# LeonardoTemperanza/LupinPathTracer

Hardware: AMD Instinct MI355X
Metric: Msamples/sec (paths x bounces) (higher is better)
Workload: dtype f32; 1 GPU; bistro_class 3840x2160, 16 bounces, 8 spp per step, Standard integrator, software BVH (BASELINE configs[4] frame; stand-in scene for bistroexterior, SURVEY 8d); frames_in_flight=1, frames_per_wavefront=6, first_pass_stack_entries=26, traversal=binary

## Files before the change

### lupinpathtracer_amd/csrc/lupin_hip.hip

```cpp

#include <hip/hip_runtime.h>
#include <hip/hip_fp16.h>
#include <cstdio>
#include <cstdlib>
#include <cstring>
#include <cmath>
#include <string>
#include <vector>
#include <set>
#include <mutex>
#include <algorithm>
#include <atomic>

#include "lupin_stages.hpp"
#include "lupin_denoise.hpp"
#include "lupin_adaptive.hpp"
#include "lupin_internal.hpp"


static inline float host_u2f(uint32_t u) { float f; memcpy(&f, &u, 4); return f; }

static thread_local std::string g_last_error;
static int fail(int code, const std::string &msg) { g_last_error = msg; return code; }
#define HIP_TRY(expr) do { hipError_t e__ = (expr); if (e__ != hipSuccess) return fail(LUPIN_ERR_HIP, std::string(#expr) + ": " + hipGetErrorString(e__)); } while (0)
// ... 88 lines not shown

struct LupinDoubleBufferedTexture
{
    LupinContext *ctx;
    LupinTexture *tex[2];
    int front_idx, back_idx;
};

struct LupinScene
{
    LupinContext *ctx;
    int device = 0;
    SceneDev dev{};
    std::vector<void *> allocations;
    uint32_t stack_entries = 1;
    uint32_t persistent_blocks[2][4] = {{0, 0, 0, 0}, {0, 0, 0, 0}};
    uint32_t wide_blocks[4] = {0, 0, 0, 0};
    uint32_t short_blocks[4] = {0, 0, 0, 0};
    bool has_wide = false;
    uint64_t leaky_triangles = 0;
    uint64_t id = 0;
    bool all_opaque = false;
    bool simple_matte = false;
    bool has_sw_bvh = false;
    bool envs_empty = true, lights_empty = true, instances_empty = true;
};

template <typename T>
static int upload(LupinScene *sc, const std::vector<T> &host, const T **out)
{
    *out = nullptr;
    size_t bytes = std::max<size_t>(host.size() * sizeof(T), sizeof(T) > 16 ? sizeof(T) : 16);
    void *d = nullptr;
    HIP_TRY(hipMalloc(&d, bytes));
    sc->allocations.push_back(d);
    HIP_TRY(hipMemsetAsync(d, 0, bytes, sc->ctx->stream));
    if (!host.empty()) HIP_TRY(hipMemcpyAsync(d, host.data(), host.size() * sizeof(T), hipMemcpyHostToDevice, sc->ctx->stream));
    *out = reinterpret_cast<const T *>(d);
    return LUPIN_OK;
}

static hipEvent_t get_event(LupinContext *ctx)
{
    if (!ctx->ev_pool.empty()) { hipEvent_t e = ctx->ev_pool.back(); ctx->ev_pool.pop_back(); return e; }
    hipEvent_t e = nullptr;
    hipEventCreate(&e);
    return e;
}

static void set_path_layout(Lane *ln, bool records)
{
    PathBuffers &pb = ln->pb;
    char *b = ln->hot;
    const size_t cap = (size_t)ln->capacity;
    pb.skey = {ln->skey, 4};
    if (records)
    {
        const uint32_t st = LP_PATH_RECORD_BYTES;
        pb.ori_rng = {b + 0, st}; pb.dir_meta = {b + 16, st}; pb.hit = {b + 32, st}; pb.hit_tri = {b + 48, st};
        pb.weight = {b + 64, st}; pb.radiance = {b + 80, st}; pb.color = {b + 96, st};
        char *m = ln->shadow;
        pb.sh_org = {m + 0, st}; pb.sh_d0 = {m + 16, st}; pb.sh_d1 = {m + 32, st}; pb.next_tri = {m + 48, st};
        pb.sh_f0 = {m + 64, st}; pb.sh_f1 = {m + 80, st}; pb.next_hit = {m + 96, st}; pb.sh_hit1 = {m + 112, st};
    }
    else
    {
        pb.ori_rng = {b, 16}; pb.dir_meta = {b + 16 * cap, 16}; pb.hit = {b + 32 * cap, 16}; pb.weight = {b + 48 * cap, 16};
        pb.radiance = {b + 64 * cap, 16}; pb.color = {b + 80 * cap, 16}; pb.hit_tri = {b + 96 * cap, 4};
        char *m = ln->shadow;
        pb.sh_org = {m, 16}; pb.sh_d0 = {m + 16 * cap, 16}; pb.sh_d1 = {m + 32 * cap, 16}; pb.sh_f0 = {m + 48 * cap, 16};
        pb.sh_f1 = {m + 64 * cap, 16}; pb.next_hit = {m + 80 * cap, 16}; pb.sh_hit1 = {m + 96 * cap, 16}; pb.next_tri = {m + 112 * cap, 4};
    }
}

static int ensure_path_buffers(LupinContext *ctx0, Lane *ctx, uint64_t slots, uint32_t iterations)
{
    (void)ctx0;
    const uint64_t per_round = (uint64_t)LP_SHARDS * LP_BLOCK;
    slots = (slots + per_round - 1) / per_round * per_round;
    if (slots > ctx->capacity)
    {
        PathBuffers &pb = ctx->pb;
        void **ptrs[] = {(void **)&ctx->hot, (void **)&ctx->shadow, (void **)&ctx->skey, (void **)&pb.vol0, (void **)&pb.vol1, (void **)&pb.queue[0], (void **)&pb.queue[1],
                         (void **)&pb.retrace};
        size_t elem[] = {LP_PATH_RECORD_BYTES, LP_PATH_RECORD_BYTES, 4, 16, 16, 4, 4, 8};
        constexpr int NPTRS = 8;
        HIP_TRY(hipStreamSynchronize(ctx->stream));
        ctx->capacity = 0;
        ctx->pb_generation++;
        for (int k = 0; k < NPTRS; k++)
            if (*ptrs[k]) { hipFree(*ptrs[k]); *ptrs[k] = nullptr; }
        for (int k = 0; k < NPTRS; k++)
            HIP_TRY(hipMalloc(ptrs[k], (size_t)slots * elem[k]));
        for (int k = 0; k < NPTRS; k++)
            HIP_TRY(hipMemsetAsync(*ptrs[k], 0, (size_t)slots * elem[k], ctx->stream));
        ctx->capacity = slots;
    }
    if (iterations + 2 > ctx->counts_capacity)
    {
        HIP_TRY(hipStreamSynchronize(ctx->stream));
        ctx->counts_capacity = 0;
        if (ctx->pb.counts) hipFree(ctx->pb.counts);
        ctx->pb.counts = nullptr;
        ctx->pb.cursors = ctx->pb.retrace_counts = ctx->pb.retrace_cursors = nullptr;
        HIP_TRY(hipMalloc((void **)&ctx->pb.counts, LP_COUNTER_ROWS * (size_t)(iterations + 2) * LP_SHARDS * sizeof(uint32_t)));
        ctx->counts_capacity = iterations + 2;
        ctx->pb.cursors = ctx->pb.counts + (size_t)ctx->counts_capacity * LP_SHARDS;
        ctx->pb.retrace_counts = ctx->pb.cursors + 2 * (size_t)ctx->counts_capacity * LP_SHARDS;
        ctx->pb.retrace_cursors = ctx->pb.retrace_counts + 2 * (size_t)ctx->counts_capacity * LP_SHARDS;
        ctx->pb_generation++;
    }
    return LUPIN_OK;
}

static uint32_t collapse_to_wide4(const std::vector<WideNode> &bin, uint32_t root_ref, std::vector<Wide4> &out, uint32_t *out_depth = nullptr)
{
    if (out_depth) *out_depth = 0;
    if (root_ref & REF_LEAF) return root_ref;
    struct Child { float lo[3], hi[3]; uint32_t ref; bool leaky, closed; };
    auto children_of = [&](uint32_t b, Child &l, Child &r) {
        const WideNode &w = bin[b];
        l.lo[0] = w.a.x; l.lo[1] = w.a.z; l.lo[2] = w.b.x; l.hi[0] = w.b.z; l.hi[1] = w.c.x; l.hi[2] = w.c.z; l.ref = w.d.x;
        r.lo[0] = w.a.y; r.lo[1] = w.a.w; r.lo[2] = w.b.y; r.hi[0] = w.b.w; r.hi[1] = w.c.y; r.hi[2] = w.c.w; r.ref = w.d.y;
        l.leaky = (w.d.z & 1u) != 0; r.leaky = (w.d.z & 2u) != 0;
        l.closed = r.closed = false;
    };
    auto inside = [](const Child &in, const Child &out) {
        for (int ax = 0; ax < 3; ax++)
            if (!(in.lo[ax] >= out.lo[ax] && in.hi[ax] <= out.hi[ax])) return false;
        return true;
    };
    auto area = [](const Child &c) {
        const double ex = (double)c.hi[0] - c.lo[0], ey = (double)c.hi[1] - c.lo[1], ez = (double)c.hi[2] - c.lo[2];
        const double a = ex * ey + ey * ez + ez * ex;
        return a == a ? a : 0.0;
    };
    struct Item { uint32_t bin_node, wide_node, depth; };
    std::vector<Item> todo;
    const uint32_t root = (uint32_t)out.size();
    out.emplace_back();
    todo.push_back({root_ref, root, 1u});
    const float nanf_ = std::nanf("");
    while (!todo.empty())
    {
        const Item it = todo.back();
        todo.pop_back();
        if (out_depth) *out_depth = std::max(*out_depth, it.depth);
        Child c[4];
        int n = 2;
        children_of(it.bin_node, c[0], c[1]);
        while (n < 4)
        {
            int pick = -1;
            double best = -1.0;
            for (int k = 0; k < n; k++)
                if (!(c[k].ref & REF_LEAF) && !c[k].closed) { const double a = area(c[k]); if (a > best) { best = a; pick = k; } }
            if (pick < 0) break;
            Child l, r;
            children_of(c[pick].ref, l, r);
            if (!inside(l, c[pick]) || !inside(r, c[pick])) { c[pick].closed = true; continue; }
            c[pick] = l;
            c[n++] = r;
        }
        Wide4 w;
        float *lo[3] = {&w.lox.x, &w.loy.x, &w.loz.x}, *hi[3] = {&w.hix.x, &w.hiy.x, &w.hiz.x};
        uint32_t refs[4];
        for (int k = 0; k < 4; k++)
        {
            for (int ax = 0; ax < 3; ax++) { lo[ax][k] = k < n ? c[k].lo[ax] : nanf_; hi[ax][k] = k < n ? c[k].hi[ax] : nanf_; }
// ... 256 lines not shown
template <int TYPE, int MODE>
static void launch_persistent_tracer(LupinContext *ctx, Lane *ln, const LupinScene *scene, const Shape &sh, uint32_t iter)
{
    hipStream_t st = ln->stream;
    const FrameParams *fp = ln->d_fp;
    unsigned long long *work = ln->work_counters, *wide = ln->wide_counters;
    {
        if (sh.wblocks)
        {
            if (ctx->counting)
            {
                hipLaunchKernelGGL((k_extend_persistent<TYPE, false, MODE, true, true, false>), dim3(sh.wblocks), dim3(LP_BLOCK), sh.wlds, st,
                                   scene->dev, fp, ln->pb, iter, ln->stat_counters, LP_REFILL_MIN, sh.wstack_words, LP_NODE_STEPS, work, wide);
                hipLaunchKernelGGL((k_extend_persistent<TYPE, false, MODE, true, false, true>), dim3(sh.pblocks), dim3(LP_BLOCK), sh.lds, st,
                                   scene->dev, fp, ln->pb, iter, ln->stat_counters, LP_REFILL_MIN, sh.stack_words, LP_NODE_STEPS, work, wide);
            }
            else
            {
                hipLaunchKernelGGL((k_extend_persistent<TYPE, false, MODE, false, true, false>), dim3(sh.wblocks), dim3(LP_BLOCK), sh.wlds, st,
                                   scene->dev, fp, ln->pb, iter, ln->stat_counters, LP_REFILL_MIN, sh.wstack_words, LP_NODE_STEPS, work, wide);
                hipLaunchKernelGGL((k_extend_persistent<TYPE, false, MODE, false, false, true>), dim3(sh.pblocks), dim3(LP_BLOCK), sh.lds, st,
                                   scene->dev, fp, ln->pb, iter, ln->stat_counters, LP_REFILL_MIN, sh.stack_words, LP_NODE_STEPS, work, wide);
            }
            return;
        }
    }
    if (sh.sblocks && !ctx->counting)
    {
        hipLaunchKernelGGL((k_extend_persistent<TYPE, false, MODE, false, false, false, true>), dim3(sh.sblocks), dim3(LP_BLOCK), sh.slds, st,
                           scene->dev, fp, ln->pb, iter, ln->stat_counters, LP_REFILL_MIN, sh.sstack_words, LP_NODE_STEPS, work, wide);
        hipLaunchKernelGGL((k_extend_persistent<TYPE, false, MODE, false, false, true>), dim3(sh.pblocks), dim3(LP_BLOCK), sh.lds, st,
                           scene->dev, fp, ln->pb, iter, ln->stat_counters, LP_REFILL_MIN, sh.stack_words, LP_NODE_STEPS, work, wide);
        return;
    }
    if (ctx->counting)
        hipLaunchKernelGGL((k_extend_persistent<TYPE, false, MODE, true>), dim3(sh.pblocks), dim3(LP_BLOCK), sh.lds, st,
                           scene->dev, fp, ln->pb, iter, ln->stat_counters, LP_REFILL_MIN, sh.stack_words, LP_NODE_STEPS, work, wide);
    else
        hipLaunchKernelGGL((k_extend_persistent<TYPE, false, MODE, false>), dim3(sh.pblocks), dim3(LP_BLOCK), sh.lds, st,
                           scene->dev, fp, ln->pb, iter, ln->stat_counters, LP_REFILL_MIN, sh.stack_words, LP_NODE_STEPS, work, wide);
}

template <int TYPE, bool LDSGEO>
static void launch_iteration_t(LupinContext *ctx, Lane *ln, const LupinScene *scene, const Shape &sh, uint32_t iter)
{
    const uint32_t blocks = sh.blocks, pblocks = sh.pblocks, stack_words = sh.stack_words;
    const size_t lds = sh.lds;
    hipStream_t st = ln->stream;
    const FrameParams *fp = ln->d_fp;
    hipEvent_t e0 = nullptr, e1 = nullptr, e2 = nullptr;
    if (ctx->timing) { e0 = get_event(ctx); e1 = get_event(ctx); e2 = get_event(ctx); hipEventRecord(e0, st); }
    const bool persistent = pblocks != 0;
    unsigned long long *work = ln->work_counters;
    if constexpr (!LDSGEO)
    {
        if (ctx->verify_wide && scene->has_wide)
            hipLaunchKernelGGL(k_verify_wide<0>, dim3(blocks), dim3(LP_BLOCK), std::max(lds, (size_t)ctx->wide_stack_pairs * 2u * LP_BLOCK * sizeof(uint32_t)), st,
                               scene->dev, fp, ln->pb, iter, ctx->wide_stack_pairs, ln->wide_counters + 2);
    }
    bool traced = false;
    if constexpr (!LDSGEO) { if (persistent) { launch_persistent_tracer<TYPE, 0>(ctx, ln, scene, sh, iter); traced = true; } }
    if (!traced)
    {
        const bool opaque = scene->all_opaque && ctx->specialize_simple;
        if (ctx->counting)
        {
            if (opaque) hipLaunchKernelGGL((k_extend<TYPE, LDSGEO, true, true>), dim3(blocks), dim3(LP_BLOCK), lds, st, scene->dev, fp, ln->pb, iter, ln->stat_counters, stack_words, work);
            else hipLaunchKernelGGL((k_extend<TYPE, LDSGEO, false, true>), dim3(blocks), dim3(LP_BLOCK), lds, st, scene->dev, fp, ln->pb, iter, ln->stat_counters, stack_words, work);
        }
        else if (opaque)
            hipLaunchKernelGGL((k_extend<TYPE, LDSGEO, true, false>), dim3(blocks), dim3(LP_BLOCK), lds, st, scene->dev, fp, ln->pb, iter, ln->stat_counters, stack_words, work);
        else
            hipLaunchKernelGGL((k_extend<TYPE, LDSGEO, false, false>), dim3(blocks), dim3(LP_BLOCK), lds, st, scene->dev, fp, ln->pb, iter, ln->stat_counters, stack_words, work);
    }
    if (ctx->timing) hipEventRecord(e1, st);
    if (ctx->debug_sync)
    {
        hipError_t de = hipStreamSynchronize(st);
        fprintf(stderr, "[lupin] iteration %u type %d: extend done: %s\n", iter, TYPE, hipGetErrorString(de)); fflush(stderr);
    }
    bool light_stage = false;
    if constexpr (TYPE == LUPIN_PATHTRACE_STANDARD || TYPE == LUPIN_PATHTRACE_MIS) light_stage = use_light_stage(ctx, scene, TYPE);
    SceneDev shade_dev = scene->dev;
    if (scene->dev.sort_shade && scene->dev.num_instances)
    {
        const uint32_t windows = ((blocks / LP_SHARDS) * LP_BLOCK + LP_SORT_WINDOW - 1) / LP_SORT_WINDOW;
        if (TYPE == LUPIN_PATHTRACE_STANDARD && persistent)
            hipLaunchKernelGGL((k_sort_queue<true, true>), dim3(windows * LP_SHARDS), dim3(LP_BLOCK), 0, st, scene->dev, ln->pb, iter);
        else
            hipLaunchKernelGGL((k_sort_queue<TYPE == LUPIN_PATHTRACE_STANDARD, false>), dim3(windows * LP_SHARDS), dim3(LP_BLOCK), 0, st, scene->dev, ln->pb, iter);
        shade_dev.sort_shade = 0;
    }
    if (scene->simple_matte && ctx->specialize_simple)
        hipLaunchKernelGGL((k_shade<TYPE, LDSGEO, true>), dim3(blocks), dim3(LP_BLOCK), lds, st, shade_dev, fp, ln->pb, iter, ln->stat_counters, stack_words);
    else if (!light_stage)
        hipLaunchKernelGGL((k_shade<TYPE, LDSGEO, false>), dim3(blocks), dim3(LP_BLOCK), lds, st, shade_dev, fp, ln->pb, iter, ln->stat_counters, stack_words);
    if constexpr (TYPE == LUPIN_PATHTRACE_STANDARD)
    {
        if (light_stage)
        {
            const size_t shade_lds = LDSGEO ? lds : std::min(lds, (size_t)LP_BLOCK * sizeof(uint32_t));
            hipLaunchKernelGGL((k_shade<TYPE, LDSGEO, false, true>), dim3(blocks), dim3(LP_BLOCK), shade_lds, st, shade_dev, fp, ln->pb, iter, ln->stat_counters, stack_words);
            hipLaunchKernelGGL((k_light_pdf<TYPE, LDSGEO>), dim3(blocks), dim3(LP_BLOCK), lds, st, scene->dev, fp, ln->pb, iter, stack_words);
        }
    }
    if constexpr (TYPE == LUPIN_PATHTRACE_MIS)
    {
        if (light_stage)
        {
            hipLaunchKernelGGL((k_shade<TYPE, LDSGEO, false, true>), dim3(blocks), dim3(LP_BLOCK), lds, st, shade_dev, fp, ln->pb, iter, ln->stat_counters, stack_words);
            hipLaunchKernelGGL((k_light_pdf_mis<LDSGEO>), dim3(blocks), dim3(LP_BLOCK), lds, st, scene->dev, fp, ln->pb, iter, stack_words);
        }
    }
    if constexpr (TYPE == LUPIN_PATHTRACE_MIS || TYPE == LUPIN_PATHTRACE_DIRECT)
    {
        bool pretraced = false;
        if constexpr (!LDSGEO)
        {
            if (persistent && ctx->persistent_shadow)
            {
                if (ctx->verify_wide && scene->has_wide)
                    hipLaunchKernelGGL(k_verify_wide<1>, dim3(blocks), dim3(LP_BLOCK), std::max(lds, (size_t)ctx->wide_stack_pairs * 2u * LP_BLOCK * sizeof(uint32_t)), st,
                                       scene->dev, fp, ln->pb, iter, ctx->wide_stack_pairs, ln->wide_counters + 2);
                launch_persistent_tracer<TYPE, 1>(ctx, ln, scene, sh, iter);
                hipLaunchKernelGGL((k_shadow<TYPE, false, true>), dim3(blocks), dim3(LP_BLOCK), lds, st, scene->dev, fp, ln->pb, iter, stack_words);
                pretraced = true;
            }
        }
        if (pretraced) {}
        else
            hipLaunchKernelGGL((k_shadow<TYPE, LDSGEO, false>), dim3(blocks), dim3(LP_BLOCK), lds, st, scene->dev, fp, ln->pb, iter, stack_words);
    }
    if (ctx->debug_sync)
    {
        fprintf(stderr, "[lupin] iteration %u type %d: stages launched, syncing\n", iter, TYPE); fflush(stderr);
        hipError_t de = hipStreamSynchronize(st);
        fprintf(stderr, "[lupin] iteration %u: %s\n", iter, hipGetErrorString(de)); fflush(stderr);
    }
    if (ctx->timing)
    {
        hipEventRecord(e2, st);
        ctx->ev_extend.push_back({e0, e1});
        ctx->ev_shade.push_back({e1, e2});
    }
    ctx->extend_launches++;
}

template <int TYPE>
static void launch_iteration(LupinContext *ctx, Lane *ln, const LupinScene *scene, bool lds_geo, const Shape &sh, uint32_t iter)
{
    if (lds_geo) launch_iteration_t<TYPE, true>(ctx, ln, scene, sh, iter);
    else launch_iteration_t<TYPE, false>(ctx, ln, scene, sh, iter);
}

static hipError_t enqueue_wavefront(LupinContext *ctx, Lane *ln, const LupinScene *scene, uint32_t pathtrace_type, bool lds_geo, uint32_t n,
                                    const Shape &sh, uint32_t iterations, const AdaptiveDev *ad = nullptr)
{
    const uint32_t blocks = sh.blocks;
    hipStream_t st = ln->stream;
    hipError_t e = hipMemsetAsync(ln->pb.counts, 0, LP_COUNTER_ROWS * (size_t)ln->counts_capacity * LP_SHARDS * sizeof(uint32_t), st);
    if (e != hipSuccess) return e;
    if (ad)
        hipLaunchKernelGGL(k_begin_adaptive, dim3(blocks), dim3(LP_BLOCK), 0, st, (const FrameParams *)ln->d_fp, ln->pb, n,
                           (const uint8_t *)ad->block_active, (const uint32_t *)ad->frames, ad->blocks_x);
    else
        hipLaunchKernelGGL(k_begin, dim3(blocks), dim3(LP_BLOCK), 0, st, (const FrameParams *)ln->d_fp, ln->pb, n);
    for (uint32_t it = 0; it < iterations; it++)
    {
        switch (pathtrace_type)
        {
        case LUPIN_PATHTRACE_STANDARD: launch_iteration<LUPIN_PATHTRACE_STANDARD>(ctx, ln, scene, lds_geo, sh, it); break;
        case LUPIN_PATHTRACE_MIS: launch_iteration<LUPIN_PATHTRACE_MIS>(ctx, ln, scene, lds_geo, sh, it); break;
        case LUPIN_PATHTRACE_NAIVE: launch_iteration<LUPIN_PATHTRACE_NAIVE>(ctx, ln, scene, lds_geo, sh, it); break;
        default: launch_iteration<LUPIN_PATHTRACE_DIRECT>(ctx, ln, scene, lds_geo, sh, it); break;
        }
    }
    return hipSuccess;
}

// ... 63 lines not shown
    int n = lupin_hip_device_count();
    if (n <= 0) return fail(LUPIN_ERR_NO_DEVICE, "no HIP device visible; this library has no CPU fallback");
    if (device_ordinal < 0 || device_ordinal >= n) return fail(LUPIN_ERR_INVALID_ARGUMENT, "device ordinal out of range");
    HIP_TRY(hipSetDevice(device_ordinal));
    LupinRuntimeInfo ri;
    lupin_hip_runtime_info(&ri);
    if (ri.num_hip_runtimes_mapped > 1)
        return fail(LUPIN_ERR_HIP, std::string("two HIP runtimes are mapped into this process (") + ri.hip_runtime_paths +
                                   "): load liblupin_hip.so in a process that has not imported another copy (e.g. a PyTorch wheel's)");
    LupinContext *ctx = new LupinContext();
    { std::lock_guard<std::mutex> lock(g_live_mu); g_live_contexts.insert(ctx); }
    ctx->device = device_ordinal;
    ctx->runtime_version = ri.runtime_hip_version;
    hipError_t e = hipSuccess;
    const char *nl = getenv("LUPIN_LANES");
    if (nl) { ctx->num_lanes = std::min(LP_MAX_LANES, std::max(1, atoi(nl))); ctx->lanes_from_env = true; }
    for (int k = 0; k < ctx->num_lanes && e == hipSuccess; k++)
    {
        Lane &ln = ctx->lanes[k];
        e = hipStreamCreateWithFlags(&ln.stream, hipStreamNonBlocking);
        if (e == hipSuccess) e = hipEventCreateWithFlags(&ln.done, hipEventDisableTiming);
        if (e == hipSuccess) e = hipMalloc((void **)&ln.d_fp, LP_MAX_BATCH * sizeof(FrameParams));
        if (e == hipSuccess) e = hipMalloc((void **)&ln.stat_counters, 2 * LP_SHARDS * sizeof(unsigned long long));
        if (e == hipSuccess) e = hipMemsetAsync(ln.stat_counters, 0, 2 * LP_SHARDS * sizeof(unsigned long long), ln.stream);
        if (e == hipSuccess) e = hipMalloc((void **)&ln.work_counters, LP_WORK_WORDS * sizeof(unsigned long long));
        if (e == hipSuccess) e = hipMemsetAsync(ln.work_counters, 0, LP_WORK_WORDS * sizeof(unsigned long long), ln.stream);
        if (e == hipSuccess) e = hipMalloc((void **)&ln.wide_counters, LP_WIDE_WORDS * sizeof(unsigned long long));
        if (e == hipSuccess) e = hipMemsetAsync(ln.wide_counters, 0, LP_WIDE_WORDS * sizeof(unsigned long long), ln.stream);
    }
    if (e == hipSuccess) e = hipEventCreateWithFlags(&ctx->marker, hipEventDisableTiming);
    if (e != hipSuccess)
    {
        lupin_hip_destroy_context(ctx);
        return fail(LUPIN_ERR_HIP, std::string("context setup: ") + hipGetErrorString(e));
    }
    ctx->stream = ctx->lanes[0].stream;
    const char *ext = getenv("LUPIN_EXTEND");
    if (ext && strcmp(ext, "persistent") == 0) ctx->persistent_extend = 1;
    else if (ext && strcmp(ext, "simple") == 0) ctx->persistent_extend = 0;
    const char *lg = getenv("LUPIN_LDS_GEOMETRY");
    ctx->lds_geometry = !(lg && strcmp(lg, "0") == 0);
    hipDeviceProp_t prop;
    if (hipGetDeviceProperties(&prop, device_ordinal) == hipSuccess && prop.multiProcessorCount > 0)
    {
        ctx->num_cus = (uint32_t)prop.multiProcessorCount;
    }
    const char *dbs = getenv("LUPIN_DEBUG_SYNC");
    ctx->debug_sync = dbs && strcmp(dbs, "0") != 0;
    if (const char *lsg = getenv("LUPIN_LIGHT_STAGE")) ctx->light_stage = atoi(lsg) != 0 ? 1 : 0;
    if (const char *pr = getenv("LUPIN_PATH_RECORDS")) ctx->path_records = atoi(pr) != 0 ? 1 : 0;
    const char *ssh = getenv("LUPIN_SIMPLE_SHADE");
    if (ssh && strcmp(ssh, "0") == 0) ctx->specialize_simple = false;
    const char *gr = getenv("LUPIN_GRAPH");
    if (gr) ctx->use_graph = strcmp(gr, "0") != 0;
    if (ctx->use_graph && ctx->runtime_version / 100000 != HIP_VERSION / 100000)
    {
        lupin_hip_destroy_context(ctx);
        return fail(LUPIN_ERR_HIP, "LUPIN_GRAPH=1 needs the HIP runtime this library was built against (built " + std::to_string(HIP_VERSION) +
                                   ", running on " + std::to_string(ri.runtime_hip_version) + ")");
    }
    const char *shd = getenv("LUPIN_SHADOW");
    if (shd && strcmp(shd, "simple") == 0) ctx->persistent_shadow = false;
    if (const char *bf = getenv("LUPIN_BATCH")) ctx->batch_frames = (uint32_t)std::min((int)LP_MAX_BATCH, std::max(0, atoi(bf)));
    if (const char *tv = getenv("LUPIN_TRAVERSAL")) ctx->wide_traversal = strcmp(tv, "wide") == 0;
    if (const char *vw = getenv("LUPIN_VERIFY_WIDE")) ctx->verify_wide = atoi(vw) != 0;
    if (const char *ss = getenv("LUPIN_SHORT_STACK")) ctx->short_stack = (uint32_t)std::max(0, atoi(ss));
    *out_ctx = ctx;
    return LUPIN_OK;
}

void lupin_hip_destroy_context(LupinContext *ctx)
{
    if (!ctx) return;
    {
        std::lock_guard<std::mutex> lock(g_live_mu);
        if (!g_live_contexts.erase(ctx)) return;
    }
    hipSetDevice(ctx->device);
    sync_all(ctx);
    for (int k = 0; k < LP_MAX_LANES; k++)
    {
        PathBuffers &pb = ctx->lanes[k].pb;
        void *ptrs[] = {ctx->lanes[k].hot, ctx->lanes[k].shadow, ctx->lanes[k].skey, pb.vol0, pb.vol1, pb.queue[0], pb.queue[1], pb.counts, ctx->lanes[k].stat_counters,
                        ctx->lanes[k].work_counters, ctx->lanes[k].wide_counters, pb.retrace};
        for (void *p : ptrs) if (p) hipFree(p);
        if (ctx->lanes[k].done) hipEventDestroy(ctx->lanes[k].done);
        if (ctx->lanes[k].graph_exec) hipGraphExecDestroy(ctx->lanes[k].graph_exec);
        if (ctx->lanes[k].graph) hipGraphDestroy(ctx->lanes[k].graph);
        if (ctx->lanes[k].d_fp) hipFree(ctx->lanes[k].d_fp);
    }
    if (ctx->marker) hipEventDestroy(ctx->marker);
    for (auto &pr : ctx->ev_extend) { hipEventDestroy(pr.first); hipEventDestroy(pr.second); }
    for (auto &pr : ctx->ev_shade) { hipEventDestroy(pr.first); hipEventDestroy(pr.second); }
    for (auto &pr : ctx->ev_total) { hipEventDestroy(pr.first); hipEventDestroy(pr.second); }
    for (auto e : ctx->ev_pool) hipEventDestroy(e);
    for (int k = 0; k < LP_MAX_LANES; k++) if (ctx->lanes[k].stream) hipStreamDestroy(ctx->lanes[k].stream);
    delete ctx;
}

int lupin_hip_sync(LupinContext *ctx)
{
    CTX_ALIVE_TRY(ctx);
    if (!ctx) return fail(LUPIN_ERR_INVALID_ARGUMENT, "ctx is null");
    HIP_TRY(hipSetDevice(ctx->device));
    HIP_TRY(sync_all(ctx));
    return LUPIN_OK;
}

int lupin_hip_set_f16_store_rounding(LupinContext *ctx, int mode)
{
    CTX_ALIVE_TRY(ctx);
    if (ctx) { int frc = flush_pending(ctx); if (frc != LUPIN_OK) return frc; }
    if (!ctx || (mode != 0 && mode != 1)) return fail(LUPIN_ERR_INVALID_ARGUMENT, "mode must be 0 (toward zero) or 1 (nearest even)");
    ctx->store_rounding = mode;
    return LUPIN_OK;
}

static uint32_t frames_per_wavefront(const LupinContext *ctx, uint64_t pixels)
{
    uint64_t k = ctx->batch_frames ? ctx->batch_frames : (pixels <= (4ull << 20) ? 16u : 8u);
    if (pixels) k = std::min<uint64_t>(k, (uint64_t)QUEUE_SLOT_MASK / pixels);
    return (uint32_t)std::max<uint64_t>(k, 1);
}

int lupin_hip_set_batch_frames(LupinContext *ctx, uint32_t frames)
{
    CTX_ALIVE_TRY(ctx);
    if (!ctx || frames > LP_MAX_BATCH) return fail(LUPIN_ERR_INVALID_ARGUMENT, "frames per wavefront must be in [1, 16] (0: chosen by dispatch size)");
    int frc = flush_pending(ctx);
    if (frc != LUPIN_OK) return frc;
    ctx->batch_frames = frames;
    return LUPIN_OK;
}

int lupin_hip_set_traversal(LupinContext *ctx, int mode)
{
    CTX_ALIVE_TRY(ctx);
    if (ctx) { int frc = flush_pending(ctx); if (frc != LUPIN_OK) return frc; }
    if (!ctx || (mode != LUPIN_TRAVERSAL_WIDE && mode != LUPIN_TRAVERSAL_BINARY)) return fail(LUPIN_ERR_INVALID_ARGUMENT, "unknown traversal mode");
    ctx->wide_traversal = mode == LUPIN_TRAVERSAL_WIDE;
    return LUPIN_OK;
}

int lupin_hip_set_accumulation_mode(LupinContext *ctx, int mode)
{
    CTX_ALIVE_TRY(ctx);
    if (ctx) { int frc = flush_pending(ctx); if (frc != LUPIN_OK) return frc; }
    if (!ctx || (mode != LUPIN_ACCUM_F16_RUNNING_AVERAGE && mode != LUPIN_ACCUM_F32)) return fail(LUPIN_ERR_INVALID_ARGUMENT, "unknown accumulation mode");
    ctx->accum_mode = mode;
    return LUPIN_OK;
}

int lupin_hip_reserve_path_state(LupinContext *ctx, uint64_t pixels, uint32_t max_bounces, uint32_t samples_per_pixel)
{
    CTX_ALIVE_TRY(ctx);
    if (pixels == 0 || pixels > (uint64_t)QUEUE_SLOT_MASK || samples_per_pixel == 0) return fail(LUPIN_ERR_INVALID_ARGUMENT, "bad path-state reservation");
    const uint32_t batch = frames_per_wavefront(ctx, pixels);
    HIP_TRY(hipSetDevice(ctx->device));
    const uint32_t iterations = samples_per_pixel * (max_bounces + 1);
    const int lanes = ctx->lanes_from_env ? ctx->num_lanes : std::min(batch > 1 ? 1 : LP_MAX_LANES, ctx->num_lanes);
    for (int k = 0; k < lanes; k++)
    {
        int rc = ensure_path_buffers(ctx, &ctx->lanes[k], pixels * batch, iterations);
        if (rc != LUPIN_OK) return rc;
    }
    return LUPIN_OK;
}
// ... 1440 lines not shown
```

### lupinpathtracer_amd/csrc/lupin_stages.hpp

```cpp
#pragma once

#include <hip/hip_runtime.h>
#include <hip/hip_fp16.h>

#include "lupin_device.hpp"
#include "../../include/lupin_tiles.h"

using namespace lpd;


constexpr uint32_t META_BOUNCE_MASK = 0xFFFu;
constexpr uint32_t META_VOLUME = 1u << 12;
constexpr uint32_t META_NEXT_EMISSION = 1u << 13;
constexpr uint32_t META_TERMINATED = 1u << 14;
constexpr uint32_t META_SAMPLE_SHIFT = 16;
constexpr uint32_t HIT_MISS = 0xFFFFFFFFu;

template <typename T>
struct PathField
{
    char *base;
    uint32_t stride;
    __device__ __forceinline__ T &operator[](size_t slot) const { return *reinterpret_cast<T *>(base + slot * stride); }
};
constexpr uint32_t LP_PATH_RECORD_BYTES = 128;

struct PathBuffers
{
    PathField<float4> ori_rng;
    PathField<float4> dir_meta;
    PathField<float4> weight;
    PathField<float4> radiance;
    PathField<float4> color;
    PathField<float4> hit;
    PathField<uint32_t> hit_tri;
    float4 *vol0;
    float4 *vol1;
    PathField<float4> next_hit;
    PathField<uint32_t> next_tri;
    PathField<float4> sh_org;
    PathField<float4> sh_d0;
    PathField<float4> sh_f0;
    PathField<float4> sh_d1;
    PathField<float4> sh_f1;
    PathField<float4> sh_hit1;
    uint32_t *queue[2];
    uint32_t *counts;
    PathField<uint32_t> skey;
    uint32_t *cursors;
    uint32_t *retrace;
    uint32_t *retrace_counts;
    uint32_t *retrace_cursors;
    uint32_t shard_cap;
};

#ifndef LP_NUM_SHARDS
#define LP_NUM_SHARDS 256
#endif
constexpr uint32_t LP_SHARDS = LP_NUM_SHARDS;

struct FrameParams
{
    LupinPushConstants pc;
    uint32_t width, height;
    uint32_t off_x, off_y;
    uint32_t reg_w, reg_h;
    uint32_t max_bounces, spp;
    uint32_t store_rne;
    uint32_t tile_px;
    uint32_t tiles_x, rank, world;
    uint32_t frame_slots;
    uint32_t num_frames;
};
constexpr uint32_t LP_MAX_BATCH = 16;

__device__ __forceinline__ uint32_t slot_frame(const FrameParams &fp, uint32_t slot, uint32_t &pixel_slot)
{
    const uint32_t frame = fp.num_frames > 1u ? slot / fp.frame_slots : 0u;
    pixel_slot = slot - frame * fp.frame_slots;
    return frame;
}


LP_FN void camera_ray(const FrameParams &fp, uint32_t gx, uint32_t gy, uint32_t &rng, f3 &ori, f3 &dir)
{
    const LupinPushConstants &pc = fp.pc;
    float j0 = rnd(rng), j1 = rnd(rng);
    float offx = j0 - 0.5f, offy = j1 - 0.5f;
    float resx = (float)fp.width, resy = (float)fp.height;
    float pcx = (float)gx + 0.5f, pcy = (resy - (float)gy) + 0.5f;
    float uvx = (pcx + offx) / resx, uvy = (pcy + offy) / resy;

    float lens = pc.camera_lens, film = pc.camera_film, aspect = pc.camera_aspect;
    float focus = pc.camera_focus, aperture = pc.camera_aperture;
    float fsx = (aspect >= 1.0f) ? film : film * aspect;
    float fsy = (aspect >= 1.0f) ? film / aspect : film;
    float d0 = rnd(rng), d1 = rnd(rng);
    float dr = sqrtf(d1);
    float ds, dc;
    lpm_sincosf(2.0f * LP_PI * d0, &ds, &dc);
    float lux = dc * dr, luy = ds * dr;

    f3 e, d;
    if (pc.flags & LUPIN_FLAG_CAMERA_ORTHO)
    {
        float sc = 1.0f / lens;
        f3 q = mk3(fsx * (0.5f - uvx) * sc, fsy * (0.5f - uvy) * sc, lens);
        e = add(mk3(-q.x, -q.y, 0.0f), mk3(lux * aperture / 2.0f, luy * aperture / 2.0f, 0.0f));
        f3 p = mk3(-q.x, -q.y, -focus);
        d = mul(normalize3(sub(p, e)), mk3(1.0f, 1.0f, -1.0f));
    }
    else
    {
        f3 q = mk3(fsx * (0.5f - uvx), fsy * (0.5f - uvy), lens);
        f3 look_at = neg(normalize3(q));
        e = mk3(lux * (aperture / 2.0f), luy * (aperture / 2.0f), 0.0f);
        f3 focus_point = divs(scale(look_at, focus), fabsf(look_at.z));
        d = mul(normalize3(sub(focus_point, e)), mk3(1.0f, 1.0f, -1.0f));
    }
    const float (*m)[4] = pc.camera_transform.m;
    ori = mk3(m[0][0] * e.x + m[1][0] * e.y + m[2][0] * e.z + m[3][0] * 1.0f,
              m[0][1] * e.x + m[1][1] * e.y + m[2][1] * e.z + m[3][1] * 1.0f,
              m[0][2] * e.x + m[1][2] * e.y + m[2][2] * e.z + m[3][2] * 1.0f);
    dir = normalize3(mk3(m[0][0] * d.x + m[1][0] * d.y + m[2][0] * d.z + m[3][0] * 0.0f,
                         m[0][1] * d.x + m[1][1] * d.y + m[2][1] * d.z + m[3][1] * 0.0f,
                         m[0][2] * d.x + m[1][2] * d.y + m[2][2] * d.z + m[3][2] * 0.0f));
}

__device__ __forceinline__ void slot_to_pixel(const FrameParams &fp, uint32_t slot, uint32_t &gx, uint32_t &gy)
{
    if (fp.tile_px)
// ... 937 lines not shown

    ShadowRays sh;
    sh.pb = (TYPE == LUPIN_PATHTRACE_MIS || TYPE == LUPIN_PATHTRACE_DIRECT) ? &pb : nullptr;
    sh.slot = slot;
    sh.flags = 0u;
    bool cont = integrate_vertex<TYPE, Geo, SIMPLE, DEFER>(geo, sc, stack, fp, p, hitrec, hit_tri, sh);
    const bool vol_dirty = p.in_medium && !was_in_medium;
    if (DEFER && cont && p.pending)
    {
        if (vol_dirty)
        {
            pb.vol0[slot] = make_float4(p.medium.density.x, p.medium.density.y, p.medium.density.z, p.medium.anisotropy);
            pb.vol1[slot] = make_float4(p.medium.scattering.x, p.medium.scattering.y, p.medium.scattering.z, 0.0f);
        }
        if (was_in_medium) pb.weight[slot] = make_float4(p.weight.x, p.weight.y, p.weight.z, 0.0f);
        if (p.radiance.x != r4.x || p.radiance.y != r4.y || p.radiance.z != r4.z)
            pb.radiance[slot] = make_float4(p.radiance.x, p.radiance.y, p.radiance.z, 0.0f);
        pb.sh_f0[slot] = make_float4(p.pend_f.x, p.pend_f.y, p.pend_f.z, p.pend_bp);
        const uint32_t nm = ((uint32_t)p.bounce & META_BOUNCE_MASK) | (p.in_medium ? META_VOLUME : 0u) |
                            (p.next_emission ? META_NEXT_EMISSION : 0u) | (sample << META_SAMPLE_SHIFT);
        pb.ori_rng[slot] = make_float4(p.ori.x, p.ori.y, p.ori.z, __uint_as_float(p.rng));
        pb.dir_meta[slot] = make_float4(p.dir.x, p.dir.y, p.dir.z, __uint_as_float(nm));
        return SLOT_WAITS_FOR_LIGHT_PDF;
    }
    if (cont)
    {
        p.bounce++;
        if (p.bounce > (int)fp.max_bounces) cont = false;
    }

    if (TYPE == LUPIN_PATHTRACE_MIS || TYPE == LUPIN_PATHTRACE_DIRECT)
    {
        if (vol_dirty)
        {
            pb.vol0[slot] = make_float4(p.medium.density.x, p.medium.density.y, p.medium.density.z, p.medium.anisotropy);
            pb.vol1[slot] = make_float4(p.medium.scattering.x, p.medium.scattering.y, p.medium.scattering.z, 0.0f);
        }
        pb.weight[slot] = make_float4(p.weight.x, p.weight.y, p.weight.z, 0.0f);
        pb.radiance[slot] = make_float4(p.radiance.x, p.radiance.y, p.radiance.z, 0.0f);
        const uint32_t nm = ((uint32_t)p.bounce & META_BOUNCE_MASK) | (p.in_medium ? META_VOLUME : 0u) |
                            (p.next_emission ? META_NEXT_EMISSION : 0u) | (cont ? 0u : META_TERMINATED) | (sample << META_SAMPLE_SHIFT);
        pb.ori_rng[slot] = make_float4(p.ori.x, p.ori.y, p.ori.z, __uint_as_float(p.rng));
        pb.dir_meta[slot] = make_float4(p.dir.x, p.dir.y, p.dir.z, __uint_as_float(nm));
        pb.sh_org[slot].w = __uint_as_float(sh.flags);
        return SLOT_ALIVE;
    }
    return path_epilogue<TYPE>(fp, fpp, pb, slot, p, sample, cont, vol_dirty, r4) ? SLOT_ALIVE : SLOT_DONE;
}

template <int TYPE, typename Geo>
__device__ __forceinline__ bool light_pdf_path(const Geo &geo, const SceneDev &sc, uint32_t *stack, const FrameParams &fp, const FrameParams *fpp, PathBuffers &pb, uint32_t slot)
{
    const float4 orr = pb.ori_rng[slot], dm = pb.dir_meta[slot], w4 = pb.weight[slot], pd = pb.sh_f0[slot];
    const uint32_t meta = __float_as_uint(dm.w);
    PathRegs p;
    p.ori = mk3(orr.x, orr.y, orr.z);
    p.dir = mk3(dm.x, dm.y, dm.z);
    p.weight = mk3(w4.x, w4.y, w4.z);
    p.rng = __float_as_uint(orr.w);
    p.bounce = (int)(meta & META_BOUNCE_MASK);
    p.in_medium = (meta & META_VOLUME) != 0;
    p.next_emission = (meta & META_NEXT_EMISSION) != 0;
    p.pending = false;
    const uint32_t sample = meta >> META_SAMPLE_SHIFT;

    const float prob = 0.5f * pd.w + 0.5f * lights_pdf(geo, sc, stack, p.ori, p.dir, fp.pc.ray_epsilon);
    p.weight = mul(p.weight, divs(mk3(pd.x, pd.y, pd.z), prob));
    bool cont = weight_checks_and_roulette(p);
    if (cont)
    {
        p.bounce++;
        if (p.bounce > (int)fp.max_bounces) cont = false;
    }
    float4 r4 = make_float4(0.0f, 0.0f, 0.0f, 0.0f);
    if (!cont) r4 = pb.radiance[slot];
    p.radiance = mk3(r4.x, r4.y, r4.z);
    return path_epilogue<TYPE>(fp, fpp, pb, slot, p, sample, cont, false, r4);
}

#ifndef LP_SORT_WINDOW
#define LP_SORT_WINDOW 4096
#endif
template <bool PEEK_COIN, bool FROM_TRACER>
__global__ void __launch_bounds__(LP_BLOCK) k_sort_queue(SceneDev sc, PathBuffers pb, uint32_t iter)
{
    constexpr uint32_t PER_THREAD = LP_SORT_WINDOW / LP_BLOCK;
    constexpr uint32_t NUM_KEYS = LP_SORT_KEYS;
    __shared__ uint32_t sorted[LP_SORT_WINDOW];
    __shared__ uint32_t bins[NUM_KEYS];
    const uint32_t shard = blockIdx.x % LP_SHARDS;
    const uint32_t count = pb.counts[iter * LP_SHARDS + shard];
    const uint32_t base_i = (blockIdx.x / LP_SHARDS) * LP_SORT_WINDOW;
    if (base_i >= count) return;
    uint32_t *entries = pb.queue[iter & 1] + (size_t)shard * pb.shard_cap + base_i;
    const uint32_t valid = min(LP_SORT_WINDOW, count - base_i);
    if (threadIdx.x < NUM_KEYS) bins[threadIdx.x] = 0u;
    __syncthreads();
    uint32_t my_slot[PER_THREAD], my_key[PER_THREAD], my_rank[PER_THREAD];
    #pragma unroll
    for (uint32_t r = 0; r < PER_THREAD; r++) my_slot[r] = entries[min(r * LP_BLOCK + threadIdx.x, valid - 1u)];
    if constexpr (FROM_TRACER)
    {
        #pragma unroll
        for (uint32_t r = 0; r < PER_THREAD; r++) my_key[r] = pb.skey[my_slot[r]] & (NUM_KEYS - 1u);
    }
    else
    {
        uint32_t hit_w[PER_THREAD], meta_w[PER_THREAD], rng_w[PER_THREAD], flags_w[PER_THREAD];
        #pragma unroll
        for (uint32_t r = 0; r < PER_THREAD; r++)
        {
            hit_w[r] = __float_as_uint(pb.hit[my_slot[r]].w);
            meta_w[r] = __float_as_uint(pb.dir_meta[my_slot[r]].w);
            rng_w[r] = PEEK_COIN ? __float_as_uint(pb.ori_rng[my_slot[r]].w) : 0u;
        }
        #pragma unroll
        for (uint32_t r = 0; r < PER_THREAD; r++) flags_w[r] = sc.instances[hit_w[r] == HIT_MISS ? 0u : hit_w[r]].flags;
        #pragma unroll
        for (uint32_t r = 0; r < PER_THREAD; r++) my_key[r] = shade_sort_key<PEEK_COIN>((meta_w[r] & META_VOLUME) != 0, hit_w[r] == HIT_MISS, flags_w[r], rng_w[r]);
    }
    #pragma unroll
    for (uint32_t r = 0; r < PER_THREAD; r++)
    {
        my_rank[r] = 0u;
        if (r * LP_BLOCK + threadIdx.x < valid) my_rank[r] = atomicAdd(&bins[my_key[r]], 1u);
    }
    __syncthreads();
    if (threadIdx.x < 64)
    {
        const uint32_t c = bins[threadIdx.x];
        uint32_t incl = c;
        for (int off = 1; off < 64; off <<= 1) { const uint32_t v = (uint32_t)__shfl_up((int)incl, off); if ((int)threadIdx.x >= off) incl += v; }
        bins[threadIdx.x] = incl - c;
    }
    __syncthreads();
    #pragma unroll
    for (uint32_t r = 0; r < PER_THREAD; r++)
        if (r * LP_BLOCK + threadIdx.x < valid) sorted[bins[my_key[r]] + my_rank[r]] = my_slot[r];
    __syncthreads();
    #pragma unroll
    for (uint32_t r = 0; r < PER_THREAD; r++)
    {
        const uint32_t j = r * LP_BLOCK + threadIdx.x;
        if (j < valid) entries[j] = sorted[j];
    }
}

template <int TYPE, bool LDSGEO, bool SIMPLE, bool DEFER = false>
__global__ void __attribute__((amdgpu_waves_per_eu(TYPE == 1 ? (DEFER ? LP_MIS_DEFER_SHADE_WAVES : LP_MIS_SHADE_WAVES) : (SIMPLE ? LP_SIMPLE_SHADE_WAVES : (DEFER ? LP_DEFER_SHADE_WAVES : LP_SHADE_WAVES)), 8))) __launch_bounds__(LP_BLOCK) k_shade(SceneDev sc, const FrameParams *__restrict__ fpp, PathBuffers pb, uint32_t iter,
                                                    unsigned long long *shard_stats, uint32_t stack_words)
{
    const FrameParams fp = *fpp;
    if (SIMPLE) sc.num_envs = 0;
    extern __shared__ __attribute__((aligned(16))) uint32_t lds_stack[];
    const auto geo = make_geo<LDSGEO>(sc, lds_stack, stack_words);
    const uint32_t shard = blockIdx.x % LP_SHARDS;
    const uint32_t count = pb.counts[iter * LP_SHARDS + shard];
    const uint32_t i = (blockIdx.x / LP_SHARDS) * LP_BLOCK + threadIdx.x;
    int state = SLOT_DONE;
    bool mine = i < count;
    uint32_t slot = 0;
    if (mine) slot = pb.queue[iter & 1][(size_t)shard * pb.shard_cap + i];
    if (mine)
    {
        const float4 orr = pb.ori_rng[slot];
        state = shade_path<TYPE, typename GeoOf<LDSGEO>::type, SIMPLE, DEFER>(geo, sc, lds_stack, fp, fpp, pb, slot, orr, pb.dir_meta[slot], __float_as_uint(orr.w), pb.hit[slot], pb.hit_tri[slot]);
    }
    if (i == 0 && iter == 0) shard_stats[shard * 2 + 1] += (unsigned long long)count * fp.spp;
    if (TYPE == LUPIN_PATHTRACE_MIS || TYPE == LUPIN_PATHTRACE_DIRECT) return;
    if (DEFER)
    {
        if (i < count) pb.queue[iter & 1][(size_t)shard * pb.shard_cap + i] = mine ? (slot | ((uint32_t)state << QUEUE_STATE_SHIFT)) : QUEUE_ENTRY_NONE;
        return;
    }
    queue_append(state == SLOT_ALIVE, slot, pb.queue[(iter + 1) & 1] + (size_t)shard * pb.shard_cap, &pb.counts[(iter + 1) * LP_SHARDS + shard]);
}

template <int TYPE, bool LDSGEO>
__global__ void __attribute__((amdgpu_waves_per_eu(LP_LIGHT_PDF_WAVES, 8))) __launch_bounds__(LP_BLOCK) k_light_pdf(SceneDev sc, const FrameParams *__restrict__ fpp, PathBuffers pb, uint32_t iter, uint32_t stack_words)
{
    const FrameParams fp = *fpp;
    extern __shared__ __attribute__((aligned(16))) uint32_t lds_stack[];
    __shared__ uint32_t waiting[LP_BLOCK];
    __shared__ uint32_t entry_slot[LP_BLOCK];
    __shared__ uint32_t verdict[LP_BLOCK];
    __shared__ uint32_t wave_total[LP_BLOCK / 64];
    const auto geo = make_geo<LDSGEO>(sc, lds_stack, stack_words);
    const uint32_t shard = blockIdx.x % LP_SHARDS;
    const uint32_t count = pb.counts[iter * LP_SHARDS + shard];
    const uint32_t i = (blockIdx.x / LP_SHARDS) * LP_BLOCK + threadIdx.x;
    if ((blockIdx.x / LP_SHARDS) * LP_BLOCK >= count) return;
    uint32_t *entries = pb.queue[iter & 1] + (size_t)shard * pb.shard_cap + (size_t)(blockIdx.x / LP_SHARDS) * LP_BLOCK;
    const uint32_t entry = i < count ? entries[threadIdx.x] : QUEUE_ENTRY_NONE;
    const uint32_t state = entry == QUEUE_ENTRY_NONE ? (uint32_t)SLOT_DONE : entry >> QUEUE_STATE_SHIFT;
    const uint32_t slot = entry & QUEUE_SLOT_MASK;
    const bool waits = state == (uint32_t)SLOT_WAITS_FOR_LIGHT_PDF;
    const unsigned long long wmask = __ballot(waits);
    const uint32_t wave = threadIdx.x >> 6, lane = threadIdx.x & 63;
    if (lane == 0) wave_total[wave] = (uint32_t)__popcll(wmask);
    verdict[threadIdx.x] = 0u;
    entry_slot[threadIdx.x] = slot;
    __syncthreads();
    uint32_t before = 0, total = 0;
    for (uint32_t w = 0; w < LP_BLOCK / 64; w++) { const uint32_t c = wave_total[w]; if (w < wave) before += c; total += c; }
    if (waits) waiting[before + (uint32_t)__popcll(wmask & ((1ull << lane) - 1ull))] = threadIdx.x;
    __syncthreads();
    if (threadIdx.x < total)
    {
        const uint32_t w = waiting[threadIdx.x];
        if (light_pdf_path<TYPE, typename GeoOf<LDSGEO>::type>(geo, sc, lds_stack, fp, fpp, pb, entry_slot[w])) verdict[w] = 1u;
    }
    __syncthreads();
    const bool alive = state == (uint32_t)SLOT_ALIVE || (waits && verdict[threadIdx.x] != 0u);
    queue_append(alive, slot, pb.queue[(iter + 1) & 1] + (size_t)shard * pb.shard_cap, &pb.counts[(iter + 1) * LP_SHARDS + shard]);
}

template <bool LDSGEO>
__global__ void __attribute__((amdgpu_waves_per_eu(LP_LIGHT_PDF_MIS_WAVES, 8))) __launch_bounds__(LP_BLOCK) k_light_pdf_mis(SceneDev sc, const FrameParams *__restrict__ fpp, PathBuffers pb, uint32_t iter, uint32_t stack_words)
{
    const FrameParams fp = *fpp;
    extern __shared__ __attribute__((aligned(16))) uint32_t lds_stack[];
    __shared__ uint32_t items[2 * LP_BLOCK];
    __shared__ uint32_t entry_slot[LP_BLOCK], entry_flags[LP_BLOCK];
    __shared__ uint32_t wave_total[LP_BLOCK / 64];
    const auto geo = make_geo<LDSGEO>(sc, lds_stack, stack_words);
    const uint32_t shard = blockIdx.x % LP_SHARDS;
    const uint32_t count = pb.counts[iter * LP_SHARDS + shard];
    const uint32_t i = (blockIdx.x / LP_SHARDS) * LP_BLOCK + threadIdx.x;
    if ((blockIdx.x / LP_SHARDS) * LP_BLOCK >= count) return;
    uint32_t slot = 0, flags = 0;
    if (i < count)
    {
        slot = pb.queue[iter & 1][(size_t)shard * pb.shard_cap + i];
        flags = __float_as_uint(pb.sh_org[slot].w) & 3u;
    }
    entry_slot[threadIdx.x] = slot;
    entry_flags[threadIdx.x] = flags;
    const uint32_t mine = (flags & 1u) + (flags >> 1);
    const uint32_t wave = threadIdx.x >> 6, lane = threadIdx.x & 63;
    uint32_t incl = mine;
    for (int off = 1; off < 64; off <<= 1) { const uint32_t v = (uint32_t)__shfl_up((int)incl, off); if ((int)lane >= off) incl += v; }
    if (lane == 63) wave_total[wave] = incl;
    __syncthreads();
    uint32_t before = incl - mine, total = 0;
    for (uint32_t w = 0; w < LP_BLOCK / 64; w++) { const uint32_t c = wave_total[w]; if (w < wave) before += c; total += c; }
    if (flags & 1u) items[before] = 2u * threadIdx.x;
    if (flags & 2u) items[before + (flags & 1u)] = 2u * threadIdx.x + 1u;
    __syncthreads();
    for (uint32_t j = threadIdx.x; j < total; j += LP_BLOCK)
    {
        const uint32_t it = items[j], t = it >> 1, k = it & 1u;
        const uint32_t s = entry_slot[t];
        const float4 so = pb.sh_org[s];
        float4 *rec = &(k ? pb.sh_d1 : pb.sh_d0)[s];
        const float4 dd = *rec;
// ... 587 lines not shown
```

Measured before the change: 1537 Msamples/s.

## Sort shade queue as index permutation and compact survivors in original order

The shade-key sort no longer rewrites the queue in material order. It writes a separate permutation array, and shading reads its work through that permutation. Shade writes each survivor or a NONE marker back to the path's original queue position, and a new compaction kernel then builds the next-iteration queue in the original (spatially coherent) order. The intent is to keep material-coherent shading while keeping the extend queue in ray-coherent order for traversal. The cost is an extra buffer, an extra kernel launch, and indirect reads.

```diff
diff --git a/lupinpathtracer_amd/csrc/lupin_hip.hip b/lupinpathtracer_amd/csrc/lupin_hip.hip
--- a/lupinpathtracer_amd/csrc/lupin_hip.hip
+++ b/lupinpathtracer_amd/csrc/lupin_hip.hip
@@ -194,9 +194,9 @@
     {
         PathBuffers &pb = ctx->pb;
         void **ptrs[] = {(void **)&ctx->hot, (void **)&ctx->shadow, (void **)&ctx->skey, (void **)&pb.vol0, (void **)&pb.vol1, (void **)&pb.queue[0], (void **)&pb.queue[1],
-                         (void **)&pb.retrace};
-        size_t elem[] = {LP_PATH_RECORD_BYTES, LP_PATH_RECORD_BYTES, 4, 16, 16, 4, 4, 8};
-        constexpr int NPTRS = 8;
+                         (void **)&pb.retrace, (void **)&pb.shade_order};
+        size_t elem[] = {LP_PATH_RECORD_BYTES, LP_PATH_RECORD_BYTES, 4, 16, 16, 4, 4, 8, 4};
+        constexpr int NPTRS = 9;
         HIP_TRY(hipStreamSynchronize(ctx->stream));
         ctx->capacity = 0;
         ctx->pb_generation++;
@@ -619,19 +619,23 @@
     bool light_stage = false;
     if constexpr (TYPE == LUPIN_PATHTRACE_STANDARD || TYPE == LUPIN_PATHTRACE_MIS) light_stage = use_light_stage(ctx, scene, TYPE);
     SceneDev shade_dev = scene->dev;
+    shade_dev.sort_shade = 0;
+    const uint32_t windows = ((blocks / LP_SHARDS) * LP_BLOCK + LP_SORT_WINDOW - 1) / LP_SORT_WINDOW;
+    const uint32_t sort_in_place = TYPE == LUPIN_PATHTRACE_MIS || TYPE == LUPIN_PATHTRACE_DIRECT;
     if (scene->dev.sort_shade && scene->dev.num_instances)
     {
-        const uint32_t windows = ((blocks / LP_SHARDS) * LP_BLOCK + LP_SORT_WINDOW - 1) / LP_SORT_WINDOW;
         if (TYPE == LUPIN_PATHTRACE_STANDARD && persistent)
-            hipLaunchKernelGGL((k_sort_queue<true, true>), dim3(windows * LP_SHARDS), dim3(LP_BLOCK), 0, st, scene->dev, ln->pb, iter);
+            hipLaunchKernelGGL((k_sort_queue<true, true>), dim3(windows * LP_SHARDS), dim3(LP_BLOCK), 0, st, scene->dev, ln->pb, iter, sort_in_place);
         else
-            hipLaunchKernelGGL((k_sort_queue<TYPE == LUPIN_PATHTRACE_STANDARD, false>), dim3(windows * LP_SHARDS), dim3(LP_BLOCK), 0, st, scene->dev, ln->pb, iter);
-        shade_dev.sort_shade = 0;
+            hipLaunchKernelGGL((k_sort_queue<TYPE == LUPIN_PATHTRACE_STANDARD, false>), dim3(windows * LP_SHARDS), dim3(LP_BLOCK), 0, st, scene->dev, ln->pb, iter, sort_in_place);
+        shade_dev.sort_shade = 1;
     }
     if (scene->simple_matte && ctx->specialize_simple)
         hipLaunchKernelGGL((k_shade<TYPE, LDSGEO, true>), dim3(blocks), dim3(LP_BLOCK), lds, st, shade_dev, fp, ln->pb, iter, ln->stat_counters, stack_words);
     else if (!light_stage)
         hipLaunchKernelGGL((k_shade<TYPE, LDSGEO, false>), dim3(blocks), dim3(LP_BLOCK), lds, st, shade_dev, fp, ln->pb, iter, ln->stat_counters, stack_words);
+    if (TYPE != LUPIN_PATHTRACE_MIS && TYPE != LUPIN_PATHTRACE_DIRECT && shade_dev.sort_shade && !light_stage)
+        hipLaunchKernelGGL(k_compact_queue, dim3(windows * LP_SHARDS), dim3(LP_BLOCK), 0, st, ln->pb, iter);
     if constexpr (TYPE == LUPIN_PATHTRACE_STANDARD)
     {
         if (light_stage)
@@ -861,7 +865,7 @@
     {
         PathBuffers &pb = ctx->lanes[k].pb;
         void *ptrs[] = {ctx->lanes[k].hot, ctx->lanes[k].shadow, ctx->lanes[k].skey, pb.vol0, pb.vol1, pb.queue[0], pb.queue[1], pb.counts, ctx->lanes[k].stat_counters,
-                        ctx->lanes[k].work_counters, ctx->lanes[k].wide_counters, pb.retrace};
+                        ctx->lanes[k].work_counters, ctx->lanes[k].wide_counters, pb.retrace, pb.shade_order};
         for (void *p : ptrs) if (p) hipFree(p);
         if (ctx->lanes[k].done) hipEventDestroy(ctx->lanes[k].done);
         if (ctx->lanes[k].graph_exec) hipGraphExecDestroy(ctx->lanes[k].graph_exec);
diff --git a/lupinpathtracer_amd/csrc/lupin_stages.hpp b/lupinpathtracer_amd/csrc/lupin_stages.hpp
--- a/lupinpathtracer_amd/csrc/lupin_stages.hpp
+++ b/lupinpathtracer_amd/csrc/lupin_stages.hpp
@@ -47,6 +47,7 @@
     uint32_t *queue[2];
     uint32_t *counts;
     PathField<uint32_t> skey;
+    uint32_t *shade_order;
     uint32_t *cursors;
     uint32_t *retrace;
     uint32_t *retrace_counts;
@@ -1150,7 +1151,7 @@
 #define LP_SORT_WINDOW 4096
 #endif
 template <bool PEEK_COIN, bool FROM_TRACER>
-__global__ void __launch_bounds__(LP_BLOCK) k_sort_queue(SceneDev sc, PathBuffers pb, uint32_t iter)
+__global__ void __launch_bounds__(LP_BLOCK) k_sort_queue(SceneDev sc, PathBuffers pb, uint32_t iter, uint32_t in_place)
 {
     constexpr uint32_t PER_THREAD = LP_SORT_WINDOW / LP_BLOCK;
     constexpr uint32_t NUM_KEYS = LP_SORT_KEYS;
@@ -1161,6 +1162,7 @@
     const uint32_t base_i = (blockIdx.x / LP_SHARDS) * LP_SORT_WINDOW;
     if (base_i >= count) return;
     uint32_t *entries = pb.queue[iter & 1] + (size_t)shard * pb.shard_cap + base_i;
+    uint32_t *order = in_place ? entries : pb.shade_order + (size_t)shard * pb.shard_cap + base_i;
     const uint32_t valid = min(LP_SORT_WINDOW, count - base_i);
     if (threadIdx.x < NUM_KEYS) bins[threadIdx.x] = 0u;
     __syncthreads();
@@ -1204,14 +1206,61 @@
     __syncthreads();
     #pragma unroll
     for (uint32_t r = 0; r < PER_THREAD; r++)
-        if (r * LP_BLOCK + threadIdx.x < valid) sorted[bins[my_key[r]] + my_rank[r]] = my_slot[r];
+        if (r * LP_BLOCK + threadIdx.x < valid) sorted[bins[my_key[r]] + my_rank[r]] = in_place ? my_slot[r] : base_i + r * LP_BLOCK + threadIdx.x;
     __syncthreads();
     #pragma unroll
     for (uint32_t r = 0; r < PER_THREAD; r++)
     {
         const uint32_t j = r * LP_BLOCK + threadIdx.x;
-        if (j < valid) entries[j] = sorted[j];
-    }
+        if (j < valid) order[j] = sorted[j];
+    }
+}
+
+__global__ void __launch_bounds__(LP_BLOCK) k_compact_queue(PathBuffers pb, uint32_t iter)
+{
+    constexpr uint32_t PER_THREAD = LP_SORT_WINDOW / LP_BLOCK;
+    static_assert(PER_THREAD % 4 == 0, "a thread reads its entries as uint4");
+    __shared__ uint32_t wave_total[LP_BLOCK / 64];
+    __shared__ uint32_t window_base;
+    const uint32_t shard = blockIdx.x % LP_SHARDS;
+    const uint32_t count = pb.counts[iter * LP_SHARDS + shard];
+    const uint32_t base_i = (blockIdx.x / LP_SHARDS) * LP_SORT_WINDOW;
+    if (base_i >= count) return;
+    const uint32_t valid = min(LP_SORT_WINDOW, count - base_i);
+    const uint32_t *entries = pb.queue[iter & 1] + (size_t)shard * pb.shard_cap + base_i;
+    const uint32_t first = threadIdx.x * PER_THREAD;
+    uint32_t e[PER_THREAD];
+    if (first + PER_THREAD <= valid)
+    {
+        #pragma unroll
+        for (uint32_t r = 0; r < PER_THREAD / 4; r++)
+        {
+            const uint4 v = reinterpret_cast<const uint4 *>(entries + first)[r];
+            e[4 * r] = v.x; e[4 * r + 1] = v.y; e[4 * r + 2] = v.z; e[4 * r + 3] = v.w;
+        }
+    }
+    else
+    {
+        #pragma unroll
+        for (uint32_t r = 0; r < PER_THREAD; r++) e[r] = first + r < valid ? entries[first + r] : QUEUE_ENTRY_NONE;
+    }
+    uint32_t mine = 0;
+    #pragma unroll
+    for (uint32_t r = 0; r < PER_THREAD; r++) mine += e[r] != QUEUE_ENTRY_NONE ? 1u : 0u;
+    const uint32_t wave = threadIdx.x >> 6, lane = threadIdx.x & 63;
+    uint32_t incl = mine;
+    for (int off = 1; off < 64; off <<= 1) { const uint32_t v = (uint32_t)__shfl_up((int)incl, off); if ((int)lane >= off) incl += v; }
+    if (lane == 63) wave_total[wave] = incl;
+    __syncthreads();
+    uint32_t before = incl - mine, total = 0;
+    for (uint32_t w = 0; w < LP_BLOCK / 64; w++) { const uint32_t c = wave_total[w]; if (w < wave) before += c; total += c; }
+    if (total == 0) return;
+    if (threadIdx.x == 0) window_base = atomicAdd(&pb.counts[(iter + 1) * LP_SHARDS + shard], total);
+    __syncthreads();
+    uint32_t *out = pb.queue[(iter + 1) & 1] + (size_t)shard * pb.shard_cap + window_base + before;
+    #pragma unroll
+    for (uint32_t r = 0; r < PER_THREAD; r++)
+        if (e[r] != QUEUE_ENTRY_NONE) *out++ = e[r];
 }
 
 template <int TYPE, bool LDSGEO, bool SIMPLE, bool DEFER = false>
@@ -1225,10 +1274,13 @@
     const uint32_t shard = blockIdx.x % LP_SHARDS;
     const uint32_t count = pb.counts[iter * LP_SHARDS + shard];
     const uint32_t i = (blockIdx.x / LP_SHARDS) * LP_BLOCK + threadIdx.x;
+    constexpr bool PERMUTED = TYPE != LUPIN_PATHTRACE_MIS && TYPE != LUPIN_PATHTRACE_DIRECT;
+    uint32_t *const entries = pb.queue[iter & 1] + (size_t)shard * pb.shard_cap;
     int state = SLOT_DONE;
     bool mine = i < count;
-    uint32_t slot = 0;
-    if (mine) slot = pb.queue[iter & 1][(size_t)shard * pb.shard_cap + i];
+    uint32_t slot = 0, pos = i;
+    if (PERMUTED && mine && sc.sort_shade) pos = pb.shade_order[(size_t)shard * pb.shard_cap + i];
+    if (mine) slot = entries[pos];
     if (mine)
     {
         const float4 orr = pb.ori_rng[slot];
@@ -1236,9 +1288,15 @@
     }
     if (i == 0 && iter == 0) shard_stats[shard * 2 + 1] += (unsigned long long)count * fp.spp;
     if (TYPE == LUPIN_PATHTRACE_MIS || TYPE == LUPIN_PATHTRACE_DIRECT) return;
+    if (!SIMPLE && mine && sc.sort_shade) pos = pb.shade_order[(size_t)shard * pb.shard_cap + i];
     if (DEFER)
     {
-        if (i < count) pb.queue[iter & 1][(size_t)shard * pb.shard_cap + i] = mine ? (slot | ((uint32_t)state << QUEUE_STATE_SHIFT)) : QUEUE_ENTRY_NONE;
+        if (mine) entries[pos] = slot | ((uint32_t)state << QUEUE_STATE_SHIFT);
+        return;
+    }
+    if (sc.sort_shade)
+    {
+        if (mine) entries[pos] = state == SLOT_ALIVE ? slot : QUEUE_ENTRY_NONE;
         return;
     }
     queue_append(state == SLOT_ALIVE, slot, pb.queue[(iter + 1) & 1] + (size_t)shard * pb.shard_cap, &pb.counts[(iter + 1) * LP_SHARDS + shard]);
```

New measurement: 1609 Msamples/s (median of 6 runs). 1.05x the previous value.
